# chhylp123/hifiasm

Measured on AMD Instinct MI355X. Metric: read-pair overlaps/sec (sum ol->length / (ha_pt_gen + all-reads h_ec_lchain pass)), higher is better.
Workload: dtype u64 hashing / int32 + f64 chain scores

## Files before the change

### hifiasm_amd/api.py

```python
from __future__ import annotations

import ctypes as C
import os

import numpy as np

_HERE = os.path.dirname(os.path.abspath(__file__))
_LIB = None


SORTDBG_SEQ, SORTDBG_WAVE_LDS, SORTDBG_WAVE_GLOBAL, SORTDBG_BLOCK, SORTDBG_SELECT = range(5)


class HaoError(RuntimeError):
    pass


class Opt(C.Structure):
    _fields_ = [("k", C.c_int32), ("w", C.c_int32), ("hpc", C.c_int32), ("sample_dist", C.c_int32), ("rewin", C.c_int32),
                ("min_hist_cnt", C.c_int32), ("max_kmer_cnt", C.c_int32), ("max_n_chain", C.c_int32),
                ("high_factor", C.c_double), ("is_ont", C.c_int32), ("bf_shift", C.c_int32), ("hg_size", C.c_int64)]


class Pass(C.Structure):
# ... 28 lines not shown


class WlistDelivery(C.Structure):
    _fields_ = [("n_ol", C.c_uint64), ("n_wins", C.c_uint64), ("n_cigar", C.c_uint64), ("n_swept", C.c_uint64), ("n_replace", C.c_uint64), ("n_untraced", C.c_uint64),
                ("win_off", C.c_void_p), ("wins", C.c_void_p), ("cig_off", C.c_void_p), ("cigars", C.c_void_p)]


DELIVER_OL, DELIVER_CL, DELIVER_EXACT, DELIVER_ED, DELIVER_TRACE, DELIVER_RESCUE, DELIVER_WLIST = 1, 2, 4, 8, 16, 32, 64
PLACE_DIAG, PLACE_REF = 0, 1

ABI_SYMBOLS = [
    "hao_opt_default", "hao_create", "hao_destroy", "hao_last_error", "hao_set_reads", "hao_ft_gen", "hao_pt_gen",
    "hao_ft_cnt", "hao_pt_get", "hao_ft_table", "hao_pt_table", "hao_hist", "hao_stats", "hao_sketch_batch",
    "hao_fetch_sketch", "hao_overlap_batch", "hao_fetch_seed_hits", "hao_fetch_overlaps", "hao_batch_totals", "hao_batch_seed_path", "hao_batch_chain_path",
    "hao_stage_times", "hao_pass_default", "hao_overlap_batch_ex", "hao_set_shard", "hao_dist_unique_id", "hao_dist_init",
    "hao_loop_create", "hao_loop_destroy", "hao_dist_init_loopback", "hao_batch_digest", "hao_selftest_rocprim", "hao_selftest_big", "hao_selftest_sortbits", "hao_unpack_cigar", "hao_unpack_overlaps", "hao_overlap_batch_async", "hao_deliver_wait", "hao_unpack_hits", "hao_exact_check", "hao_fetch_exact", "hao_window_ed_batch", "hao_index_save", "hao_index_load", "hao_next_slot", "hao_attach", "hao_window_trace_batch", "hao_delivery_digest", "hao_ft_passes", "hao_ovlp_bin_read", "hao_ovlp_bin_write", "hao_window_ed_grid", "hao_fetch_ed_grid",
    "hao_deliver_ed_config", "hao_deliver_ed", "hao_unpack_ed",
    "hao_window_trace_grid", "hao_fetch_trace_grid", "hao_deliver_trace", "hao_unpack_trace",
    "hao_window_ed_ref", "hao_fetch_ed_ovlp", "hao_deliver_ed_config_ref", "hao_ref_thresholds",
    "hao_window_rescue_ref", "hao_fetch_rescue", "hao_rescue_task", "hao_deliver_rescue", "hao_unpack_rescue",
    "hao_window_wlist_ref", "hao_fetch_wlist", "hao_deliver_wlist", "hao_unpack_wlist",
    "hao_dist_gather_reads", "hao_reads_digest", "hao_index_load_dist", "hao_shard_layout",
]


RESCUE_OVLP = np.dtype([("verdict", np.uint16), ("flags", np.uint16), ("exit_win", np.uint32), ("align_length", np.uint32), ("n_rescued", np.uint32)])
RESCUE_FWD, RESCUE_BWD, RESCUE_ANCHOR, RESCUE_UNTRACED, RESCUE_NO_EXIT = 0, 1, 2, 1, 0xFFFFFFFF
WLIST_PRIMARY, WLIST_UNTRACED = 3, 1 << 19


def wlist_records(raw):
# ... 635 lines not shown
```

### hifiasm_amd/csrc/hao_capi_rest.hpp

```cpp
#pragma once

#include <atomic>
#include <new>
#include <stdexcept>
#include <thread>
extern "C" {

int hao_ft_gen(hao_ctx *c, int32_t *hom_cov)
{
	if (!c) return HAO_EINVAL;
	HAO_NOT_ON_VIEW(c, "hao_ft_gen"); ++c->index_gen;
	HIP_TRY(hipSetDevice(c->device));
	c->timer.begin(c->stream);
	int rc = hao_ft_run(c);
	if (rc != HAO_OK) return rc;
	c->timer.mark("ft_release");
	HIP_TRY(hipStreamSynchronize(c->stream));
	c->timer.collect(c->stage_ms);
	if (hom_cov) *hom_cov = c->ft_peak_hom;
	return HAO_OK;
}

int32_t hao_ft_cnt(hao_ctx *c, uint64_t y)
{
// ... 692 lines not shown
	HAO_CHECK_LAUNCH();
	HIP_TRY(hipMemcpyAsync(out, d.p, n * 8, hipMemcpyDeviceToHost, c->stream));
	if (out_kh) HIP_TRY(hipMemcpyAsync(out_kh, d.p + n, n * 8, hipMemcpyDeviceToHost, c->stream));
	HIP_TRY(hipStreamSynchronize(c->stream));
	return HAO_OK;
}

__global__ void hao_selftest_fill_kernel(uint64_t n, uint64_t *x, uint64_t *v)
{
	const uint64_t i = (uint64_t)blockIdx.x * blockDim.x + threadIdx.x;
	if (i < n) { x[i] = hao_hash64(i * 0x9E3779B97F4A7C15ULL + 12345); v[i] = i; }
}
__global__ void hao_selftest_s40_fill_kernel(uint64_t n, uint64_t *x)
{
	const uint64_t i = (uint64_t)blockIdx.x * blockDim.x + threadIdx.x;
	if (i < n) { const uint64_t g = i % (n / 5 + 1); x[i] = (hao_hash64(g + 99) & ~((1ULL << HAO_SORT40_LOWBITS) - 1)) | ((g & 255) ? 0x155ULL : ((hao_hash64(i) >> 7) & 3) * 0x2a5b7ULL); }
}
__global__ void hao_selftest_s40_cmp_kernel(const uint64_t *a, const uint64_t *b, const uint32_t *ia, const uint32_t *ib, uint64_t n, unsigned long long *bad)
{
	const uint64_t i = (uint64_t)blockIdx.x * blockDim.x + threadIdx.x;
	if (i < n && (a[i] != b[i] || ia[i] != ib[i])) atomicAdd(bad, 1ULL);
}
int hao_selftest_sortbits(hao_ctx *c, uint64_t n, uint64_t out[4])
{
	if (!c || !out || n < 16 || n >= (1ULL << 32)) return HAO_EINVAL;
	HIP_TRY(hipSetDevice(c->device));
	DevBuf<uint64_t> x, s1, s2; DevBuf<uint32_t> o, o1, o2; DevBuf<unsigned long long> bad;
	HIP_TRY(x.reserve(n)); HIP_TRY(s1.reserve(n)); HIP_TRY(s2.reserve(n)); HIP_TRY(o.reserve(n)); HIP_TRY(o1.reserve(n)); HIP_TRY(o2.reserve(n)); HIP_TRY(bad.reserve(1));
	HIP_TRY(hipMemsetAsync(bad.p, 0, 8, c->stream));
	hipLaunchKernelGGL(hao_selftest_s40_fill_kernel, dim3((unsigned)((n + 255) / 256)), dim3(256), 0, c->stream, n, x.p); HAO_CHECK_LAUNCH();
	int rc = hao_index_sort(c, x.p, s1.p, o.p, o1.p, n, false);
	if (!rc) rc = hao_index_sort(c, x.p, s2.p, o.p, o2.p, n, true);
	if (!rc) {
		hipLaunchKernelGGL(hao_selftest_s40_cmp_kernel, dim3((unsigned)((n + 255) / 256)), dim3(256), 0, c->stream, s1.p, s2.p, o1.p, o2.p, n, bad.p);
		unsigned long long hb = 0;
		if (hipMemcpyAsync(&hb, bad.p, 8, hipMemcpyDeviceToHost, c->stream) != hipSuccess || hipStreamSynchronize(c->stream) != hipSuccess) rc = HAO_ENODEV;
		out[0] = hb; for (int k = 0; k < 3; ++k) out[1 + k] = c->peeked(PK_SORT40, k);
	}
	return rc;
}

int hao_selftest_rocprim(uint64_t n, uint64_t out[2])
{
	hao_ctx tmp_ctx; hao_ctx *c = &tmp_ctx;
	if (!out || n == 0 || n >= (1ULL << 32)) return HAO_EINVAL;
	out[0] = out[1] = 0;
	hipStream_t st = nullptr;
	DevBuf<uint64_t> x, v, x2, v2, gx, gv; DevBuf<uint32_t> ok, ok2, oi, oi2; DevBuf<unsigned char> tmp;
	HIP_TRY(x.reserve(n)); HIP_TRY(v.reserve(n)); HIP_TRY(x2.reserve(n)); HIP_TRY(v2.reserve(n)); HIP_TRY(gx.reserve(n)); HIP_TRY(gv.reserve(n));
	HIP_TRY(ok.reserve(n)); HIP_TRY(ok2.reserve(n)); HIP_TRY(oi.reserve(n)); HIP_TRY(oi2.reserve(n));
	hipLaunchKernelGGL(hao_selftest_fill_kernel, dim3((unsigned)((n + 255) / 256)), dim3(256), 0, st, n, x.p, v.p);
	HIP_TRY(hipGetLastError());
	size_t tb = 0;
	HIP_TRY(rocprim::radix_sort_pairs(nullptr, tb, x.p, x2.p, v.p, v2.p, n, 48, 64, st)); HIP_TRY(tmp.reserve(tb + 256));
// ... 65 lines not shown
```

### hifiasm_amd/csrc/hao_ctx.hpp

```cpp
#pragma once
#include <time.h>
#include <rocprim/rocprim.hpp>
#include <map>
#include <algorithm>
#include <cstdlib>
#include <cstring>
#include "hao_common.cuh"
#include "hao_grid_pair.cuh"

struct hao_ctx;
static void hao_set_err(hao_ctx *c, const std::string &m);

template<typename T> struct DevBuf {
	T *p = nullptr; size_t cap = 0; bool borrowed = false;
	DevBuf() = default;
	DevBuf(const DevBuf&) = delete; DevBuf &operator=(const DevBuf&) = delete;
	DevBuf(DevBuf &&o) noexcept : p(o.p), cap(o.cap), borrowed(o.borrowed) { o.p = nullptr; o.cap = 0; o.borrowed = false; }
	DevBuf &operator=(DevBuf &&o) noexcept { if (this != &o) { release(); p = o.p; cap = o.cap; borrowed = o.borrowed; o.p = nullptr; o.cap = 0; o.borrowed = false; } return *this; }
	~DevBuf() { release(); }
	hipError_t reserve(size_t n) {
		if (n <= cap) return hipSuccess;
		if (borrowed) return hipErrorInvalidValue;
		if (p) (void)hipFree(p);
		p = nullptr; cap = 0;
// ... 23 lines not shown
	void mark(const char *name) {
		size_t i = names.size();
		if (i >= ev.size()) { hipEvent_t e; (void)hipEventCreate(&e); ev.push_back(e); }
		names.push_back(name); host_t.push_back(now()); (void)hipEventRecord(ev[i], st);
		if (hao_dbg_sync) { const hipError_t e = hipStreamSynchronize(st); fprintf(stderr, "[stage] %s: %s\n", name, hipGetErrorString(e)); fflush(stderr); }
	}
	void collect(std::vector<std::pair<std::string, float> > &out) {
		out.clear();
		for (size_t i = 1; i < names.size(); ++i) { float ms = 0; (void)hipEventElapsedTime(&ms, ev[i - 1], ev[i]); out.push_back(std::make_pair(names[i], ms)); }
		for (size_t i = 1; i < names.size(); ++i) if (names[i].compare(0, 3, "ft_") == 0) out.push_back(std::make_pair("host_" + names[i], (float)((host_t[i] - host_t[i - 1]) * 1e3)));
	}
	~StageTimer() { for (auto e : ev) (void)hipEventDestroy(e); }
};

struct hao_switches {
	bool seedphase = false, qcphase = false, dp_stats = false, selphase = false, dltime = false, bloom = false;
	bool seq_chain = false, dp_seqtail = false, dp_nospec = false, dp_serial = false, seq_prune = false, seed_noql = false;
	long long sk_gcap = -1, exc_cap = -1, ft_chunk_slots = 0; unsigned long long gather_chunk = 64ULL << 20, ix_pad = 0, sort40_min = 1ULL << 23; int fc_raw_every = 0, exc_every = 0; bool qmz_raw = false, arena_probe = false;
	int arena_numa = 3, seed_merge_maxn = 24000, seed_lds_ratio = 120, ft_passes = 0, seed_lds = 1;
	static bool in_list(const char *v, const char *name) {
		const size_t n = strlen(name);
		for (const char *p = v; p && *p; ) { const char *e = strchr(p, ','); const size_t l = e ? (size_t)(e - p) : strlen(p); if (l == n && strncmp(p, name, n) == 0) return true; p = e ? e + 1 : nullptr; }
		return false;
	}
	static bool in_kv(const char *v, const char *name, unsigned long long &out) {
		const size_t n = strlen(name);
		for (const char *p = v; p && *p; ) { const char *e = strchr(p, ','); if (strncmp(p, name, n) == 0 && p[n] == '=') { out = strtoull(p + n + 1, nullptr, 10); return true; } p = e ? e + 1 : nullptr; }
		return false;
	}
	void load() {
		if (const char *v = getenv("HAO_DBG_PRINT")) {
			seedphase = in_list(v, "seed"); qcphase = in_list(v, "qc"); dp_stats = in_list(v, "dp"); selphase = in_list(v, "sel"); dltime = in_list(v, "dl"); bloom = in_list(v, "bloom"); hao_dbg_sync = in_list(v, "sync");
		}
		if (const char *v = getenv("HAO_DBG_FORCE")) {
			seq_chain = in_list(v, "seq_chain");
			dp_seqtail = in_list(v, "dp_seqtail");
			dp_nospec = in_list(v, "dp_nospec");
			dp_serial = in_list(v, "dp_serial");
			seq_prune = in_list(v, "seq_prune");
			seed_noql = in_list(v, "noql");
		}
		if (const char *v = getenv("HAO_DBG_TEST")) {
			unsigned long long x;
			if (in_kv(v, "ix_pad", x)) ix_pad = x;
			if (in_kv(v, "sort40_min", x)) sort40_min = x;
			if (in_kv(v, "sk_gcap", x)) sk_gcap = (long long)x;
			if (in_kv(v, "exc_cap", x)) exc_cap = (long long)x;
			if (in_kv(v, "fc_raw_every", x)) fc_raw_every = (int)x;
			if (in_kv(v, "exc_every", x)) exc_every = (int)x;
			if (in_kv(v, "qmz_raw", x)) qmz_raw = x != 0;
			if (in_kv(v, "arena_probe", x)) arena_probe = x != 0;
			if (in_kv(v, "ft_chunk_slots", x)) ft_chunk_slots = (long long)x;
			if (in_kv(v, "gather_chunk", x)) gather_chunk = std::max<unsigned long long>(x, 64);
		}
		if (const char *e = getenv("HAO_SEED_LDS")) seed_lds = atoi(e) ? 1 : 0;
		if (const char *e = getenv("HAO_SEED_LDS_RATIO")) seed_lds_ratio = std::max(0, atoi(e));
		if (const char *e = getenv("HAO_SEED_MERGE_MAXN")) seed_merge_maxn = std::max(0, atoi(e));
		if (const char *e = getenv("HAO_FT_PASSES")) ft_passes = std::max(0, atoi(e));
		if (const char *e = getenv("HAO_ARENA_NUMA")) arena_numa = atoi(e);
	}
// ... 83 lines not shown
	DevBuf<uint8_t> d_scalar_flag; DevBuf<uint32_t> d_scalar_list, d_unit_rid;
	DevBuf<uint64_t> d_pool_x, d_pool_info; DevBuf<uint32_t> d_pool_ord; DevBuf<unsigned long long> d_cursor; DevBuf<int> d_err;
	DevBuf<uint64_t> d_chunk_base, d_chunk_dst; DevBuf<uint32_t> d_chunk_cnt;
	DevBuf<uint64_t> d_g_x, d_g_info; DevBuf<uint32_t> d_g_ord; DevBuf<uint64_t> d_g_off; DevBuf<uint32_t> d_new_n; DevBuf<uint64_t> d_new_n64;
	DevBuf<uint64_t> d_mz_x, d_mz_info, d_mz_off;
	DevBuf<unsigned char> d_tmp; DevBuf<unsigned char> d_ring; DevBuf<uint32_t> d_ringord, d_cnt_ws;
	std::vector<uint64_t> h_mz_off; std::vector<hao_mz_t> h_mz_fetch;
	bool has_pt = false; int64_t pt_hist[HAO_N_COUNTS];
	uint64_t ix_n_mz = 0, ix_n_sorted = 0, ix_n_keys = 0, ix_n_pos = 0, ix_pad = 0; int ix_bucket_bits = 16;
	DevBuf<uint64_t> d_ix_mz_x, d_ix_mz_info, d_ix_mz_off;
	DevBuf<uint64_t> d_ix_sx, d_ix_sinfo;
	DevBuf<uint64_t> d_ix_lk; bool lk_valid = false; DevBuf<uint32_t> w_runid;
	DevBuf<uint64_t> d_ix_keys, d_ix_start; DevBuf<uint32_t> d_ix_cnt; DevBuf<uint32_t> d_ix_bucket;
	DevBuf<uint64_t> w_ukeys, w_flag, w_kpos, w_ustart; DevBuf<uint32_t> w_ucnt; DevBuf<unsigned long long> w_hist; DevBuf<uint32_t> w_ok, w_ok2, w_oi, w_oi2;
	DevBuf<uint32_t> w_s40_list, w_s40_o; DevBuf<uint64_t> w_s40_x, w_lkv2; DevBuf<unsigned long long> w_s40_cnt; uint64_t s40_runs = 0;
	std::vector<uint64_t> h_ix_keys, h_ix_off, h_ix_pos, h_ix_mz_off; bool h_ix_valid = false;
	WinResident win;
	DevBuf<hao_ed_task_t> al_task; DevBuf<uint64_t> al_k1, al_k2, al_path; DevBuf<uint32_t> al_i1, al_order, al_sel; DevBuf<hao_ed_result_t> al_res; DevBuf<hao_trace_result_t> al_tres;
	DevBuf<uint8_t> al_want; DevBuf<uint16_t> al_cig;
	uint32_t ded_window = 0, ded_thre = 0;
	uint32_t ded_place = 0; double ded_erate = 0; DevBuf<uint8_t> ded_tab;
	struct RefGrid {
		DevBuf<uint64_t> cnt, woff; DevBuf<int16_t> shift; DevBuf<uint8_t> werr; DevBuf<hao_ed_pair> pairs; DevBuf<unsigned long long> ctr;
	} rf;
	DevBuf<uint8_t> rf_tab; uint32_t rf_tab_wl = 0; double rf_tab_erate = 0; DevBuf<hao_ed_ovlp_sum> rf_sum; std::vector<hao_ed_ovlp_sum> rf_hsum; uint64_t rf_unres = 0, rs_wc = 0;
	struct Rescue {
		DevBuf<uint16_t> wpe; DevBuf<uint64_t> rbase, path, off; DevBuf<hao_rs_state> st; DevBuf<hao_rs_win> rec, wins; DevBuf<hao_rs_ovlp> ovlp; DevBuf<unsigned long long> ctr;
		std::vector<hao_rs_ovlp> h_ovlp; std::vector<uint64_t> h_win_off; std::vector<hao_rs_win> h_wins;
	} rs;
	uint64_t rs_slots = 0, rs_rounds = 0, rs_active = 0, rs_total = 0, rs_nw = 0;
// ... 77 lines not shown
```

### hifiasm_amd/csrc/hao_index.cuh

```cuda
#pragma once
#include "hao_common.cuh"
#include "hao_sketch.cuh"

#define HAO_KH_CHUNK 2048

struct hao_kh_args {
	const uint8_t *packed; const uint64_t *pk_off; const uint32_t *len;
	const uint64_t *tile_off; const uint32_t *tile_ord; const uint32_t *n_runs;
	const uint64_t *chunk_off; const uint8_t *scalar_flag; const uint64_t *kmer_off;
	uint64_t rid_lo, n_sel; int k, hpc; uint64_t *out;
	uint64_t ch0;
};

__global__ __launch_bounds__(256) void kmer_hash_chunk_kernel(hao_kh_args a)
{
	extern __shared__ __align__(16) unsigned char smem[];
	const int k = a.k, tid = threadIdx.x, lane = tid & 63, wv = tid >> 6;
	const int NE = HAO_KH_CHUNK + k + 1, NW = (NE + 63) / 64 + 1;
	uint64_t *pl0 = (uint64_t*)smem, *pl1 = pl0 + NW; uint8_t *rcode = (uint8_t*)(pl1 + NW);
	uint64_t ch = blockIdx.x + a.ch0, lo = 0, hi = a.n_sel;
	while (lo < hi) { uint64_t m = (lo + hi) >> 1; if (a.chunk_off[m + 1] <= ch) lo = m + 1; else hi = m; }
	const uint64_t r = lo;
	if (a.scalar_flag[r]) return;
	const uint32_t ci = (uint32_t)(ch - a.chunk_off[r]);
// ... 103 lines not shown
__global__ void hao_bucket_kernel(const uint64_t *keys, uint64_t n, int shift, uint32_t nb, uint32_t *bucket)
{
	uint32_t b = blockIdx.x * blockDim.x + threadIdx.x;
	if (b > nb) return;
	if (b == nb) { bucket[b] = (uint32_t)n; return; }
	uint64_t lo = 0, hi = n;
	while (lo < hi) { uint64_t m = (lo + hi) >> 1; if ((keys[m] >> shift) < b) lo = m + 1; else hi = m; }
	bucket[b] = (uint32_t)lo;
}

__global__ void hao_iota_kernel(uint32_t *v, uint64_t n)
{
	const uint64_t i = (uint64_t)blockIdx.x * blockDim.x + threadIdx.x;
	if (i < n) v[i] = (uint32_t)i;
}
#define HAO_SORT40_LOWBITS 24
__global__ void hao_sort40_mark_kernel(const uint64_t *sx, uint64_t m, uint32_t *list, unsigned long long *cnt, uint64_t cap)
{
	const uint64_t j = (uint64_t)blockIdx.x * blockDim.x + threadIdx.x + 1;
	if (j >= m) return;
	const uint64_t b = sx[j], a = sx[j - 1], top = b >> HAO_SORT40_LOWBITS;
	if ((a >> HAO_SORT40_LOWBITS) != top || a <= b) return;
	uint64_t i = j - 1;
	while (i > 0 && (sx[i - 1] >> HAO_SORT40_LOWBITS) == top) { if (sx[i - 1] > sx[i]) return; --i; }
	const unsigned long long k = atomicAdd(cnt, 1ULL);
	if (k < cap) list[k] = (uint32_t)i;
}
__global__ __launch_bounds__(64) void hao_sort40_fix_kernel(uint64_t *sx, uint32_t *oi, uint64_t m, const uint32_t *list, unsigned long long *cnt, uint64_t cap, uint64_t *tx, uint32_t *to, uint64_t tcap)
{
	const uint64_t n_runs = cnt[0] < cap ? cnt[0] : cap;
	if (blockIdx.x >= n_runs) return;
	const int lane = hao_lane();
	const uint64_t s = list[blockIdx.x], top = sx[s] >> HAO_SORT40_LOWBITS;
	uint64_t e = s;
	for (;;) {
		const uint64_t i = e + lane; const unsigned long long bal = __ballot(i < m && (sx[i] >> HAO_SORT40_LOWBITS) == top);
		if (bal == ~0ULL) { e += 64; continue; }
		e += (uint64_t)(__ffsll((long long)~bal) - 1); break;
	}
	const uint64_t L = e - s;
	unsigned long long base = 0;
	if (lane == 0) base = atomicAdd(cnt + 1, (unsigned long long)L);
	base = (unsigned long long)__shfl((long long)base, 0);
	if (base + L > tcap) { if (lane == 0) cnt[2] = 1; return; }
	uint64_t last = 0, out = 0; bool first = true;
	while (out < L) {
		uint64_t mn = ~0ULL;
		for (uint64_t i = s + lane; i < e; i += 64) { const uint64_t k = sx[i]; if ((first || k > last) && k < mn) mn = k; }
#pragma unroll
		for (int d = 32; d >= 1; d >>= 1) { const uint64_t o = (uint64_t)__shfl_xor((long long)mn, d); if (o < mn) mn = o; }
		for (uint64_t i0 = s; i0 < e; i0 += 64) {
// ... 15 lines not shown
	const uint32_t o = sidx[j], u = runid[j] - 1;
	sinfo[j] = info[o];
	int c = ucnt[u] > HAO_MAX_COUNT ? HAO_MAX_COUNT : (int)ucnt[u];
	lk[o] = (c >= lo && c <= hi) ? ((ustart[u] + base) | (uint64_t)c << 48) : 0;
}
__global__ void hao_index_gather_kernel(uint64_t m, const uint32_t *sidx, const uint32_t *runid, const uint32_t *ucnt, const uint64_t *ustart, int lo, int hi,
		const uint64_t *info, uint64_t *sinfo, uint64_t *val, uint64_t base)
{
	const uint64_t j = (uint64_t)blockIdx.x * blockDim.x + threadIdx.x;
	if (j >= m) return;
	const uint32_t o = sidx[j], u = runid[j] - 1;
	sinfo[j] = info[o];
	int c = ucnt[u] > HAO_MAX_COUNT ? HAO_MAX_COUNT : (int)ucnt[u];
	val[j] = (c >= lo && c <= hi) ? ((ustart[u] + base) | (uint64_t)c << 48) : 0;
}
__global__ void hao_scatter_u64_kernel(const uint64_t *in, const uint32_t *idx, uint64_t n, uint64_t *out)
{
	const uint64_t i = (uint64_t)blockIdx.x * blockDim.x + threadIdx.x;
	if (i < n) out[idx[i]] = in[i];
}

struct hao_pt_dev {
	const uint64_t *keys, *start; const uint32_t *cnt, *bucket; const uint64_t *sinfo; uint64_t n_keys; int bshift;
};

__device__ __forceinline__ uint32_t hao_pt_lookup(const hao_pt_dev &pt, uint64_t x, uint64_t *start)
{
	uint32_t b = (uint32_t)(x >> pt.bshift), lo = pt.bucket[b], hi = pt.bucket[b + 1], e = hi;
	while (lo < hi) { uint32_t m = (lo + hi) >> 1; if (pt.keys[m] < x) lo = m + 1; else hi = m; }
	if (lo < e && pt.keys[lo] == x) { *start = pt.start[lo]; return pt.cnt[lo]; }
// ... 33 lines not shown
```

### hifiasm_amd/csrc/hao_tables.hpp

```cpp
#pragma once
#include <chrono>
#include "hao_comm.hpp"
#include "hao_pipeline.hpp"
#include "hao_index.cuh"
#include "hao_host.hpp"

__global__ void hao_lower_bound_kernel(const uint64_t *keys, uint64_t n, const uint64_t *targets, int nt, uint64_t *out)
{
	int t = blockIdx.x * blockDim.x + threadIdx.x;
	if (t >= nt) return;
	uint64_t lo = 0, hi = n, x = targets[t];
	while (lo < hi) { uint64_t m = (lo + hi) >> 1; if (keys[m] < x) lo = m + 1; else hi = m; }
	out[t] = lo;
}
__global__ void hao_lower_bound_low12_kernel(const uint64_t *keys, uint64_t n, const uint64_t *targets, int nt, uint64_t *out)
{
	int t = blockIdx.x * blockDim.x + threadIdx.x;
	if (t >= nt) return;
	uint64_t lo = 0, hi = n, x = targets[t];
	while (lo < hi) { uint64_t m = (lo + hi) >> 1; if ((keys[m] & 4095) < x) lo = m + 1; else hi = m; }
	out[t] = lo;
}
__global__ void hao_owner_key_kernel(const uint64_t *x, uint64_t n, uint32_t *key, uint32_t *idx)
{
// ... 531 lines not shown
	if (int rc = hao_build_bucket(c, c->d_ft_keys.p, n_kept, 16, c->d_ft_bucket)) return rc;
	if (int rc = hao_ft_build_hash(c, n_kept)) return rc;
	HIP_TRY(hipStreamSynchronize(c->stream));
	kcnt.release(); slots.release(); chunks.release(); kmer_off.release(); kh_chunk_off.release();
	c->has_ft = true;
	{
		int mx = (int)(c->ft_peak_hom * c->opt.high_factor + .499);
		c->hom_cov = c->ft_peak_hom;
		if (c->max_n_chain < mx) c->max_n_chain = mx;
	}
	c->timer.mark("ft_table");
	return HAO_OK;
}

static inline uint64_t hao_sort40_cap(uint64_t m) { return std::max<uint64_t>(1 << 16, m >> 10); }
static int hao_index_sort(hao_ctx *c, const uint64_t *x, uint64_t *sx, uint32_t *oi, uint32_t *oi2, uint64_t m, bool sort40)
{
	hipLaunchKernelGGL(hao_iota_kernel, dim3((unsigned)((m + 255) / 256)), dim3(256), 0, c->stream, oi, m); HAO_CHECK_LAUNCH();
	const int b0 = sort40 ? HAO_SORT40_LOWBITS : 0;
	size_t tb = 0;
	HIP_TRY(rocprim::radix_sort_pairs(nullptr, tb, x, sx, oi, oi2, m, b0, 64, c->stream)); HIP_TRY(hao_tmp(c, tb));
	HIP_TRY(rocprim::radix_sort_pairs(c->d_tmp.p, tb, x, sx, oi, oi2, m, b0, 64, c->stream));
	if (sort40) {
		const uint64_t cap = hao_sort40_cap(m), tcap = 64 * cap;
		HIP_TRY(c->w_s40_list.reserve(cap)); HIP_TRY(c->w_s40_x.reserve(tcap)); HIP_TRY(c->w_s40_o.reserve(tcap)); HIP_TRY(c->w_s40_cnt.reserve(4));
		HIP_TRY(hipMemsetAsync(c->w_s40_cnt.p, 0, 32, c->stream));
		hipLaunchKernelGGL(hao_sort40_mark_kernel, dim3((unsigned)((m + 255) / 256)), dim3(256), 0, c->stream, sx, m, c->w_s40_list.p, c->w_s40_cnt.p, cap); HAO_CHECK_LAUNCH();
		hipLaunchKernelGGL(hao_sort40_fix_kernel, dim3((unsigned)cap), dim3(64), 0, c->stream, sx, oi2, m, c->w_s40_list.p, c->w_s40_cnt.p, cap, c->w_s40_x.p, c->w_s40_o.p, tcap); HAO_CHECK_LAUNCH();
		if (int rc = hao_peek(c, c->w_s40_cnt.p, 3, PK_SORT40)) return rc;
	}
	return HAO_OK;
}

static int hao_pt_run(hao_ctx *c)
{
	const uint64_t n = c->n_reads;
	c->has_pt = false; c->h_ix_valid = false; c->h_ix_mz_off.clear();
	const bool sharded = c->comm && c->comm->active();
	auto local_sketch = [&]() -> int {
		if (n == 0) { hao_set_err(c, "no reads"); return HAO_EINVAL; }
		if (int rc = hao_sketch_run(c, 0, n, c->has_ft, c->opt.sample_dist, 1)) return rc;
		std::swap(c->d_ix_mz_x, c->d_mz_x); std::swap(c->d_ix_mz_info, c->d_mz_info); std::swap(c->d_ix_mz_off, c->d_mz_off);
		HIP_TRY(c->d_mz_x.reserve_exact(c->d_ix_mz_x.cap)); HIP_TRY(c->d_mz_info.reserve_exact(c->d_ix_mz_info.cap)); HIP_TRY(c->d_mz_off.reserve_exact(c->d_ix_mz_off.cap));
// ... 20 lines not shown
		return HAO_OK;
	};
	auto peaks_and_range = [&](int *hi_out) {
		int het = -1;
		c->hom_cov = hao_find_peaks(c->pt_hist, HAO_N_COUNTS, c->opt.min_hist_cnt, &het, hao_prior_hom(c)); c->het_cov = het;
		int hi;
		if (c->has_ft) hi = HAO_MAX_COUNT - 1;
		else { hi = (int)(c->hom_cov * c->opt.high_factor); if (hi > HAO_MAX_COUNT - 1) hi = HAO_MAX_COUNT - 1; }
		*hi_out = hi;
	};
	c->lk_valid = false;
	if (!sharded) {
		const uint64_t m = c->ix_n_mz;
		if (m >= (1ULL << 32)) { hao_set_err(c, "more than 2^32 minimizers on one device"); return HAO_EUNSUPP; }
		const uint64_t pad = c->ix_pad = c->sw.ix_pad;
		HIP_TRY(c->d_ix_sx.reserve(m + 1)); HIP_TRY(c->d_ix_sinfo.reserve(m + pad + 8)); HIP_TRY(c->w_oi.reserve(m + 1)); HIP_TRY(c->w_oi2.reserve(m + 1));
		HIP_TRY(c->w_runid.reserve(m + 1)); HIP_TRY(c->d_ix_lk.reserve(m + 1));
		bool sort40 = m >= c->sw.sort40_min;
		for (;;) {
			if (m) { if (int rc = hao_index_sort(c, c->d_ix_mz_x.p, c->d_ix_sx.p, c->w_oi.p, c->w_oi2.p, m, sort40)) return rc; }
			c->ix_n_sorted = m;
			c->timer.mark("pt_sort");
			if (int rc = rle_hist(c->d_ix_sx.p, m)) return rc;
			if (m && sort40) {
				c->s40_runs = c->peeked(PK_SORT40);
				if (c->s40_runs > hao_sort40_cap(m) || c->peeked(PK_SORT40, 2)) { sort40 = false; continue; }
			}
			break;
		}
		c->timer.mark("pt_count");
		int hi; peaks_and_range(&hi);
		if (int rc = hao_keep_runs(c, ukeys.p, ucnt.p, n_unique, 2, hi, c->d_ix_keys, &c->d_ix_start, c->d_ix_cnt, &c->ix_n_keys, &c->ix_n_pos)) return rc;
		if (m) {
			auto heads = rocprim::make_transform_iterator(rocprim::make_counting_iterator<uint64_t>(0), RunHead32{c->d_ix_sx.p});
			size_t tb = 0;
			HIP_TRY(rocprim::inclusive_scan(nullptr, tb, heads, c->w_runid.p, m, rocprim::plus<uint32_t>(), c->stream)); HIP_TRY(hao_tmp(c, tb));
			HIP_TRY(rocprim::inclusive_scan(c->d_tmp.p, tb, heads, c->w_runid.p, m, rocprim::plus<uint32_t>(), c->stream));
			if (m >= c->sw.sort40_min) {
				int nb = 1; while ((1ULL << nb) < m) ++nb;
				const int b0 = nb > 8 ? nb - 8 : 0;
				HIP_TRY(c->w_lkv2.reserve(m + 1));
				hipLaunchKernelGGL(hao_index_gather_kernel, dim3((unsigned)((m + 255) / 256)), dim3(256), 0, c->stream, m, c->w_oi2.p, c->w_runid.p, ucnt.p, c->w_ustart.p, 2, hi,
								   c->d_ix_mz_info.p, c->d_ix_sinfo.p + pad, c->d_ix_sx.p, pad);
				HAO_CHECK_LAUNCH();
				size_t tb2 = 0;
				HIP_TRY(rocprim::radix_sort_pairs(nullptr, tb2, c->w_oi2.p, c->w_oi.p, c->d_ix_sx.p, c->w_lkv2.p, m, b0, nb, c->stream)); HIP_TRY(hao_tmp(c, tb2));
				HIP_TRY(rocprim::radix_sort_pairs(c->d_tmp.p, tb2, c->w_oi2.p, c->w_oi.p, c->d_ix_sx.p, c->w_lkv2.p, m, b0, nb, c->stream));
				hipLaunchKernelGGL(hao_scatter_u64_kernel, dim3((unsigned)((m + 255) / 256)), dim3(256), 0, c->stream, c->w_lkv2.p, c->w_oi.p, m, c->d_ix_lk.p);
				HAO_CHECK_LAUNCH();
			} else {
				hipLaunchKernelGGL(hao_index_finish_kernel, dim3((unsigned)((m + 255) / 256)), dim3(256), 0, c->stream, m, c->w_oi2.p, c->w_runid.p, ucnt.p, c->w_ustart.p, 2, hi,
								   c->d_ix_mz_info.p, c->d_ix_sinfo.p + pad, c->d_ix_lk.p, pad);
				HAO_CHECK_LAUNCH();
			}
			if (pad && c->ix_n_keys) { hipLaunchKernelGGL(hao_add_const_kernel, dim3((unsigned)((c->ix_n_keys + 255) / 256)), dim3(256), 0, c->stream, c->d_ix_start.p, c->ix_n_keys, pad); HAO_CHECK_LAUNCH(); }
		}
		c->lk_valid = true;
// ... 158 lines not shown
```

### include/hao.h

```cpp
#ifndef HAO_H
#define HAO_H
#include <stdint.h>

#ifdef __cplusplus
extern "C" {
#endif

#define HAO_OK          0
#define HAO_ENODEV     -1
#define HAO_EINVAL     -2
#define HAO_ENOMEM     -3
#define HAO_EUNSUPP    -4

typedef struct hao_ctx hao_ctx;

typedef struct {
	int32_t k;
	int32_t w;
	int32_t hpc;
	int32_t sample_dist;
	int32_t rewin;
	int32_t min_hist_cnt;
	int32_t max_kmer_cnt;
	int32_t max_n_chain;
// ... 199 lines not shown
int hao_index_load(hao_ctx *c, const char *prefix, int32_t *number_of_round);
int hao_index_load_dist(hao_ctx *c, const char *prefix, const uint64_t *first_rid , int32_t *number_of_round);
int hao_shard_layout(hao_ctx *c, uint64_t *n_reads, uint64_t *rid_base, uint64_t *n_total, const uint32_t **all_len);

typedef struct { uint64_t qns; uint32_t qe, tn, ts, te; uint32_t ml, rev, bl, del; uint8_t el, no_l_indel, pad[6]; } hao_ma_hit_t;
int hao_ovlp_bin_read(const char *path, uint64_t *n_reads, uint8_t **flags, uint64_t **off, hao_ma_hit_t **hits);
int hao_ovlp_bin_write(const char *path, uint64_t n_reads, const uint8_t *flags, const uint64_t *off, const hao_ma_hit_t *hits);

int hao_batch_digest(hao_ctx *c, uint64_t *out, uint64_t *out_kh);
int hao_delivery_digest(const hao_delivery_t *d, uint64_t *out, int n_threads);

int hao_selftest_rocprim(uint64_t n, uint64_t out[2]);
int hao_selftest_big(uint64_t n, uint64_t out[3]);

int hao_selftest_sortbits(hao_ctx *c, uint64_t n, uint64_t out[4]);

#define HAO_SORTDBG_SEQ 0
#define HAO_SORTDBG_WAVE_LDS 1
#define HAO_SORTDBG_WAVE_GLOBAL 2
#define HAO_SORTDBG_BLOCK 3
#define HAO_SORTDBG_SELECT 4
int hao_dbg_sort_perm(hao_ctx *c, int mode, int path, int variant, uint64_t n_arr, const uint64_t *off, const uint64_t *xs, const int32_t *sc, uint32_t *perm);

int hao_stage_times(hao_ctx *c, const char **names, float *ms, int cap);

#ifdef __cplusplus
}
#endif
#endif
```

Before: 179.7 million.

## Adaptive partial-key radix sort ladder and run-walk index gather

The index sort now picks how many low key bits to skip (32, 24 or 0) using a collision estimate taken from the previous build or the k-mer peak. If the fix-up pass overflows, it falls back one rung at a time. For large indexes with many distinct keys, a new per-run kernel assigns run info by binary search over run starts in shared memory. This replaces the inclusive scan that built run ids and the per-element gather. The aim is to cut radix passes and a full scan over all minimizers, at the risk of retries when the estimate is wrong. Selftests and debug switches are also added.

```diff
diff --git a/hifiasm_amd/api.py b/hifiasm_amd/api.py
--- a/hifiasm_amd/api.py
+++ b/hifiasm_amd/api.py
@@ -66,7 +66,7 @@
     "hao_ft_cnt", "hao_pt_get", "hao_ft_table", "hao_pt_table", "hao_hist", "hao_stats", "hao_sketch_batch",
     "hao_fetch_sketch", "hao_overlap_batch", "hao_fetch_seed_hits", "hao_fetch_overlaps", "hao_batch_totals", "hao_batch_seed_path", "hao_batch_chain_path",
     "hao_stage_times", "hao_pass_default", "hao_overlap_batch_ex", "hao_set_shard", "hao_dist_unique_id", "hao_dist_init",
-    "hao_loop_create", "hao_loop_destroy", "hao_dist_init_loopback", "hao_batch_digest", "hao_selftest_rocprim", "hao_selftest_big", "hao_selftest_sortbits", "hao_unpack_cigar", "hao_unpack_overlaps", "hao_overlap_batch_async", "hao_deliver_wait", "hao_unpack_hits", "hao_exact_check", "hao_fetch_exact", "hao_window_ed_batch", "hao_index_save", "hao_index_load", "hao_next_slot", "hao_attach", "hao_window_trace_batch", "hao_delivery_digest", "hao_ft_passes", "hao_ovlp_bin_read", "hao_ovlp_bin_write", "hao_window_ed_grid", "hao_fetch_ed_grid",
+    "hao_loop_create", "hao_loop_destroy", "hao_dist_init_loopback", "hao_batch_digest", "hao_selftest_rocprim", "hao_selftest_big", "hao_selftest_sortbits", "hao_selftest_sortladder", "hao_selftest_index_runs", "hao_unpack_cigar", "hao_unpack_overlaps", "hao_overlap_batch_async", "hao_deliver_wait", "hao_unpack_hits", "hao_exact_check", "hao_fetch_exact", "hao_window_ed_batch", "hao_index_save", "hao_index_load", "hao_next_slot", "hao_attach", "hao_window_trace_batch", "hao_delivery_digest", "hao_ft_passes", "hao_ovlp_bin_read", "hao_ovlp_bin_write", "hao_window_ed_grid", "hao_fetch_ed_grid",
     "hao_deliver_ed_config", "hao_deliver_ed", "hao_unpack_ed",
     "hao_window_trace_grid", "hao_fetch_trace_grid", "hao_deliver_trace", "hao_unpack_trace",
     "hao_window_ed_ref", "hao_fetch_ed_ovlp", "hao_deliver_ed_config_ref", "hao_ref_thresholds",
diff --git a/hifiasm_amd/csrc/hao_capi_rest.hpp b/hifiasm_amd/csrc/hao_capi_rest.hpp
--- a/hifiasm_amd/csrc/hao_capi_rest.hpp
+++ b/hifiasm_amd/csrc/hao_capi_rest.hpp
@@ -730,7 +730,7 @@
 __global__ void hao_selftest_s40_fill_kernel(uint64_t n, uint64_t *x)
 {
 	const uint64_t i = (uint64_t)blockIdx.x * blockDim.x + threadIdx.x;
-	if (i < n) { const uint64_t g = i % (n / 5 + 1); x[i] = (hao_hash64(g + 99) & ~((1ULL << HAO_SORT40_LOWBITS) - 1)) | ((g & 255) ? 0x155ULL : ((hao_hash64(i) >> 7) & 3) * 0x2a5b7ULL); }
+	if (i < n) { const uint64_t g = i % (n / 5 + 1); x[i] = (hao_hash64(g + 99) & ~((1ULL << 24) - 1)) | ((g & 255) ? 0x155ULL : ((hao_hash64(i) >> 7) & 3) * 0x2a5b7ULL); }
 }
 __global__ void hao_selftest_s40_cmp_kernel(const uint64_t *a, const uint64_t *b, const uint32_t *ia, const uint32_t *ib, uint64_t n, unsigned long long *bad)
 {
@@ -743,10 +743,11 @@
 	HIP_TRY(hipSetDevice(c->device));
 	DevBuf<uint64_t> x, s1, s2; DevBuf<uint32_t> o, o1, o2; DevBuf<unsigned long long> bad;
 	HIP_TRY(x.reserve(n)); HIP_TRY(s1.reserve(n)); HIP_TRY(s2.reserve(n)); HIP_TRY(o.reserve(n)); HIP_TRY(o1.reserve(n)); HIP_TRY(o2.reserve(n)); HIP_TRY(bad.reserve(1));
+	const uint64_t cap = hao_sort40_cap(n);
 	HIP_TRY(hipMemsetAsync(bad.p, 0, 8, c->stream));
 	hipLaunchKernelGGL(hao_selftest_s40_fill_kernel, dim3((unsigned)((n + 255) / 256)), dim3(256), 0, c->stream, n, x.p); HAO_CHECK_LAUNCH();
-	int rc = hao_index_sort(c, x.p, s1.p, o.p, o1.p, n, false);
-	if (!rc) rc = hao_index_sort(c, x.p, s2.p, o.p, o2.p, n, true);
+	int rc = hao_index_sort(c, x.p, s1.p, o.p, o1.p, n, 0, cap, 64 * cap);
+	if (!rc) rc = hao_index_sort(c, x.p, s2.p, o.p, o2.p, n, 24, cap, 64 * cap);
 	if (!rc) {
 		hipLaunchKernelGGL(hao_selftest_s40_cmp_kernel, dim3((unsigned)((n + 255) / 256)), dim3(256), 0, c->stream, s1.p, s2.p, o1.p, o2.p, n, bad.p);
 		unsigned long long hb = 0;
@@ -754,6 +755,69 @@
 		out[0] = hb; for (int k = 0; k < 3; ++k) out[1 + k] = c->peeked(PK_SORT40, k);
 	}
 	return rc;
+}
+
+__global__ void hao_selftest_ladder_fill_kernel(uint64_t n, int lowbits, uint64_t *x)
+{
+	const uint64_t i = (uint64_t)blockIdx.x * blockDim.x + threadIdx.x;
+	if (i >= n) return;
+	const uint64_t G = n / 5 + 1, g = i % G, k = i / G, top = (g * 0x9E3779B97F4A7C15ULL) & (~0ULL >> lowbits);
+	uint64_t low = 0x155;
+	if ((g & 255) == 0) { const int p = (int)((g >> 8) % 3); low = (p == 0 ? ((k & 1) ? 1 : 2) : p == 1 ? (k % 3 ? k % 3 : 3) : ((0x31524 >> (4 * k)) & 15)) * 0x2a5b7ULL; }
+	x[i] = top << lowbits | low;
+}
+int hao_selftest_sortladder(hao_ctx *c, const uint64_t *keys, uint64_t n, int lowbits, uint64_t cap, uint64_t tcap, uint64_t *out_keys, uint32_t *out_idx, uint64_t out[6])
+{
+	if (!c || !out || n < 16 || n >= (1ULL << 32) || (lowbits != 0 && lowbits != 24 && lowbits != 32) || (!keys && !lowbits)) return HAO_EINVAL;
+	HIP_TRY(hipSetDevice(c->device));
+	if (!cap) cap = hao_sort40_cap(n);
+	if (!tcap) tcap = 64 * cap;
+	if (cap >= (1ULL << 31)) return HAO_EINVAL;
+	DevBuf<uint64_t> x, s1, s2; DevBuf<uint32_t> o, o1, o2; DevBuf<unsigned long long> bad;
+	HIP_TRY(x.reserve(n)); HIP_TRY(s1.reserve(n)); HIP_TRY(s2.reserve(n)); HIP_TRY(o.reserve(n)); HIP_TRY(o1.reserve(n)); HIP_TRY(o2.reserve(n)); HIP_TRY(bad.reserve(1));
+	HIP_TRY(hipMemsetAsync(bad.p, 0, 8, c->stream));
+	if (keys) HIP_TRY(hipMemcpyAsync(x.p, keys, n * 8, hipMemcpyHostToDevice, c->stream));
+	else { hipLaunchKernelGGL(hao_selftest_ladder_fill_kernel, dim3((unsigned)((n + 255) / 256)), dim3(256), 0, c->stream, n, lowbits, x.p); HAO_CHECK_LAUNCH(); }
+	if (int rc = hao_index_sort(c, x.p, s1.p, o.p, o1.p, n, 0, cap, tcap)) return rc;
+	uint64_t retries = 0;
+	for (int k = 0; k < 4; ++k) out[k] = 0;
+	for (;;) {
+		if (int rc = hao_index_sort(c, x.p, s2.p, o.p, o2.p, n, lowbits, cap, tcap)) return rc;
+		HIP_TRY(hipStreamSynchronize(c->stream));
+		if (!lowbits) break;
+		for (int k = 0; k < 3; ++k) out[1 + k] = c->peeked(PK_SORT40, k);
+		if (!hao_sort_failed(c, cap)) break;
+		lowbits = hao_sort_next_rung(lowbits); ++retries;
+	}
+	out[4] = (uint64_t)lowbits; out[5] = retries;
+	hipLaunchKernelGGL(hao_selftest_s40_cmp_kernel, dim3((unsigned)((n + 255) / 256)), dim3(256), 0, c->stream, s1.p, s2.p, o1.p, o2.p, n, bad.p); HAO_CHECK_LAUNCH();
+	unsigned long long hb = 0;
+	HIP_TRY(hipMemcpyAsync(&hb, bad.p, 8, hipMemcpyDeviceToHost, c->stream));
+	if (out_keys) HIP_TRY(hipMemcpyAsync(out_keys, s2.p, n * 8, hipMemcpyDeviceToHost, c->stream));
+	if (out_idx) HIP_TRY(hipMemcpyAsync(out_idx, o2.p, n * 4, hipMemcpyDeviceToHost, c->stream));
+	HIP_TRY(hipStreamSynchronize(c->stream));
+	out[0] = hb;
+	return HAO_OK;
+}
+
+int hao_selftest_index_runs(hao_ctx *c, uint64_t m, uint64_t n_runs, const uint64_t *ustart, const uint32_t *ucnt, int lo, int hi, uint64_t pad, const uint32_t *sidx, const uint64_t *info,
+		uint64_t *out_sinfo, uint64_t *out_val)
+{
+	if (!c || !m || !n_runs || n_runs > m || m >= (1ULL << 32) || !ustart || !ucnt || !sidx || !info || !out_sinfo || !out_val || lo < 1 || ustart[0] != 0) return HAO_EINVAL;
+	for (uint64_t u = 0; u < n_runs; ++u) if (ustart[u] >= m || (u && ustart[u] <= ustart[u - 1])) { hao_set_err(c, "hao_selftest_index_runs: run starts do not ascend inside the positions"); return HAO_EINVAL; }
+	for (uint64_t j = 0; j < m; ++j) if (sidx[j] >= m) { hao_set_err(c, "hao_selftest_index_runs: a carried index beyond the records"); return HAO_EINVAL; }
+	HIP_TRY(hipSetDevice(c->device));
+	DevBuf<uint64_t> d_st, d_info, d_sinfo, d_val; DevBuf<uint32_t> d_cnt, d_sidx;
+	HIP_TRY(d_st.reserve(n_runs + 1)); HIP_TRY(d_cnt.reserve(n_runs + 1)); HIP_TRY(d_sidx.reserve(m)); HIP_TRY(d_info.reserve(m)); HIP_TRY(d_sinfo.reserve(m + pad)); HIP_TRY(d_val.reserve(m));
+	HIP_TRY(hipMemcpyAsync(d_st.p, ustart, n_runs * 8, hipMemcpyHostToDevice, c->stream)); HIP_TRY(hipMemcpyAsync(d_cnt.p, ucnt, n_runs * 4, hipMemcpyHostToDevice, c->stream));
+	HIP_TRY(hipMemcpyAsync(d_sidx.p, sidx, m * 4, hipMemcpyHostToDevice, c->stream)); HIP_TRY(hipMemcpyAsync(d_info.p, info, m * 8, hipMemcpyHostToDevice, c->stream));
+	HIP_TRY(hipMemsetAsync(d_sinfo.p, 0xff, (m + pad) * 8, c->stream)); HIP_TRY(hipMemsetAsync(d_val.p, 0xff, m * 8, c->stream));
+	hipLaunchKernelGGL(hao_index_runs_kernel, dim3((unsigned)((n_runs + HAO_IXR_RUNS - 1) / HAO_IXR_RUNS)), dim3(256), 0, c->stream, m, n_runs, d_sidx.p, d_cnt.p, d_st.p, lo, hi,
+					   d_info.p, d_sinfo.p + pad, d_val.p, pad);
+	HAO_CHECK_LAUNCH();
+	HIP_TRY(hipMemcpyAsync(out_sinfo, d_sinfo.p + pad, m * 8, hipMemcpyDeviceToHost, c->stream)); HIP_TRY(hipMemcpyAsync(out_val, d_val.p, m * 8, hipMemcpyDeviceToHost, c->stream));
+	HIP_TRY(hipStreamSynchronize(c->stream));
+	return HAO_OK;
 }
 
 int hao_selftest_rocprim(uint64_t n, uint64_t out[2])
diff --git a/hifiasm_amd/csrc/hao_ctx.hpp b/hifiasm_amd/csrc/hao_ctx.hpp
--- a/hifiasm_amd/csrc/hao_ctx.hpp
+++ b/hifiasm_amd/csrc/hao_ctx.hpp
@@ -61,9 +61,9 @@
 };
 
 struct hao_switches {
-	bool seedphase = false, qcphase = false, dp_stats = false, selphase = false, dltime = false, bloom = false;
+	bool seedphase = false, qcphase = false, dp_stats = false, selphase = false, dltime = false, bloom = false, sortprint = false;
 	bool seq_chain = false, dp_seqtail = false, dp_nospec = false, dp_serial = false, seq_prune = false, seed_noql = false;
-	long long sk_gcap = -1, exc_cap = -1, ft_chunk_slots = 0; unsigned long long gather_chunk = 64ULL << 20, ix_pad = 0, sort40_min = 1ULL << 23; int fc_raw_every = 0, exc_every = 0; bool qmz_raw = false, arena_probe = false;
+	long long sk_gcap = -1, exc_cap = -1, ft_chunk_slots = 0; unsigned long long gather_chunk = 64ULL << 20, ix_pad = 0, sort40_min = 1ULL << 23, ixr_min = 0; int fc_raw_every = 0, exc_every = 0, sort_lowbits = -1; bool qmz_raw = false, arena_probe = false;
 	int arena_numa = 3, seed_merge_maxn = 24000, seed_lds_ratio = 120, ft_passes = 0, seed_lds = 1;
 	static bool in_list(const char *v, const char *name) {
 		const size_t n = strlen(name);
@@ -77,7 +77,7 @@
 	}
 	void load() {
 		if (const char *v = getenv("HAO_DBG_PRINT")) {
-			seedphase = in_list(v, "seed"); qcphase = in_list(v, "qc"); dp_stats = in_list(v, "dp"); selphase = in_list(v, "sel"); dltime = in_list(v, "dl"); bloom = in_list(v, "bloom"); hao_dbg_sync = in_list(v, "sync");
+			seedphase = in_list(v, "seed"); qcphase = in_list(v, "qc"); dp_stats = in_list(v, "dp"); selphase = in_list(v, "sel"); dltime = in_list(v, "dl"); bloom = in_list(v, "bloom"); sortprint = in_list(v, "sort"); hao_dbg_sync = in_list(v, "sync");
 		}
 		if (const char *v = getenv("HAO_DBG_FORCE")) {
 			seq_chain = in_list(v, "seq_chain");
@@ -91,6 +91,8 @@
 			unsigned long long x;
 			if (in_kv(v, "ix_pad", x)) ix_pad = x;
 			if (in_kv(v, "sort40_min", x)) sort40_min = x;
+			if (in_kv(v, "sort_lowbits", x)) sort_lowbits = (int)x;
+			if (in_kv(v, "ixr_min", x)) ixr_min = x;
 			if (in_kv(v, "sk_gcap", x)) sk_gcap = (long long)x;
 			if (in_kv(v, "exc_cap", x)) exc_cap = (long long)x;
 			if (in_kv(v, "fc_raw_every", x)) fc_raw_every = (int)x;
@@ -204,6 +206,7 @@
 	DevBuf<uint64_t> d_ix_keys, d_ix_start; DevBuf<uint32_t> d_ix_cnt; DevBuf<uint32_t> d_ix_bucket;
 	DevBuf<uint64_t> w_ukeys, w_flag, w_kpos, w_ustart; DevBuf<uint32_t> w_ucnt; DevBuf<unsigned long long> w_hist; DevBuf<uint32_t> w_ok, w_ok2, w_oi, w_oi2;
 	DevBuf<uint32_t> w_s40_list, w_s40_o; DevBuf<uint64_t> w_s40_x, w_lkv2; DevBuf<unsigned long long> w_s40_cnt; uint64_t s40_runs = 0;
+	int s40_lowbits = 0; uint64_t s40_prev_m = 0, s40_prev_unique = 0;
 	std::vector<uint64_t> h_ix_keys, h_ix_off, h_ix_pos, h_ix_mz_off; bool h_ix_valid = false;
 	WinResident win;
 	DevBuf<hao_ed_task_t> al_task; DevBuf<uint64_t> al_k1, al_k2, al_path; DevBuf<uint32_t> al_i1, al_order, al_sel; DevBuf<hao_ed_result_t> al_res; DevBuf<hao_trace_result_t> al_tres;
diff --git a/hifiasm_amd/csrc/hao_index.cuh b/hifiasm_amd/csrc/hao_index.cuh
--- a/hifiasm_amd/csrc/hao_index.cuh
+++ b/hifiasm_amd/csrc/hao_index.cuh
@@ -141,27 +141,26 @@
 	const uint64_t i = (uint64_t)blockIdx.x * blockDim.x + threadIdx.x;
 	if (i < n) v[i] = (uint32_t)i;
 }
-#define HAO_SORT40_LOWBITS 24
-__global__ void hao_sort40_mark_kernel(const uint64_t *sx, uint64_t m, uint32_t *list, unsigned long long *cnt, uint64_t cap)
+__global__ void hao_sort40_mark_kernel(const uint64_t *sx, uint64_t m, uint32_t *list, unsigned long long *cnt, uint64_t cap, int lowbits)
 {
 	const uint64_t j = (uint64_t)blockIdx.x * blockDim.x + threadIdx.x + 1;
 	if (j >= m) return;
-	const uint64_t b = sx[j], a = sx[j - 1], top = b >> HAO_SORT40_LOWBITS;
-	if ((a >> HAO_SORT40_LOWBITS) != top || a <= b) return;
+	const uint64_t b = sx[j], a = sx[j - 1], top = b >> lowbits;
+	if ((a >> lowbits) != top || a <= b) return;
 	uint64_t i = j - 1;
-	while (i > 0 && (sx[i - 1] >> HAO_SORT40_LOWBITS) == top) { if (sx[i - 1] > sx[i]) return; --i; }
+	while (i > 0 && (sx[i - 1] >> lowbits) == top) { if (sx[i - 1] > sx[i]) return; --i; }
 	const unsigned long long k = atomicAdd(cnt, 1ULL);
 	if (k < cap) list[k] = (uint32_t)i;
 }
-__global__ __launch_bounds__(64) void hao_sort40_fix_kernel(uint64_t *sx, uint32_t *oi, uint64_t m, const uint32_t *list, unsigned long long *cnt, uint64_t cap, uint64_t *tx, uint32_t *to, uint64_t tcap)
+__global__ __launch_bounds__(64) void hao_sort40_fix_kernel(uint64_t *sx, uint32_t *oi, uint64_t m, const uint32_t *list, unsigned long long *cnt, uint64_t cap, uint64_t *tx, uint32_t *to, uint64_t tcap, int lowbits)
 {
 	const uint64_t n_runs = cnt[0] < cap ? cnt[0] : cap;
 	if (blockIdx.x >= n_runs) return;
 	const int lane = hao_lane();
-	const uint64_t s = list[blockIdx.x], top = sx[s] >> HAO_SORT40_LOWBITS;
+	const uint64_t s = list[blockIdx.x], top = sx[s] >> lowbits;
 	uint64_t e = s;
 	for (;;) {
-		const uint64_t i = e + lane; const unsigned long long bal = __ballot(i < m && (sx[i] >> HAO_SORT40_LOWBITS) == top);
+		const uint64_t i = e + lane; const unsigned long long bal = __ballot(i < m && (sx[i] >> lowbits) == top);
 		if (bal == ~0ULL) { e += 64; continue; }
 		e += (uint64_t)(__ffsll((long long)~bal) - 1); break;
 	}
@@ -207,6 +206,26 @@
 	int c = ucnt[u] > HAO_MAX_COUNT ? HAO_MAX_COUNT : (int)ucnt[u];
 	val[j] = (c >= lo && c <= hi) ? ((ustart[u] + base) | (uint64_t)c << 48) : 0;
 }
+#define HAO_IXR_RUNS 256
+__global__ __launch_bounds__(256) void hao_index_runs_kernel(uint64_t m, uint64_t n_runs, const uint32_t *sidx, const uint32_t *ucnt, const uint64_t *ustart, int lo, int hi,
+		const uint64_t *info, uint64_t *sinfo, uint64_t *val, uint64_t base)
+{
+	__shared__ uint64_t l_start[HAO_IXR_RUNS + 1]; __shared__ uint32_t l_cnt[HAO_IXR_RUNS];
+	const uint64_t u0 = (uint64_t)blockIdx.x * HAO_IXR_RUNS;
+	if (u0 >= n_runs) return;
+	const int R = (int)(n_runs - u0 < HAO_IXR_RUNS ? n_runs - u0 : HAO_IXR_RUNS);
+	for (int t = threadIdx.x; t <= R; t += 256) l_start[t] = u0 + t < n_runs ? ustart[u0 + t] : m;
+	for (int t = threadIdx.x; t < R; t += 256) { const int c = ucnt[u0 + t] > HAO_MAX_COUNT ? HAO_MAX_COUNT : (int)ucnt[u0 + t]; l_cnt[t] = (c >= lo && c <= hi) ? (uint32_t)c : 0u; }
+	__syncthreads();
+	const uint64_t j1 = l_start[R] < m ? l_start[R] : m;
+	for (uint64_t j = l_start[0] + threadIdx.x; j < j1; j += 256) {
+		int a = 0, b = R;
+		while (b - a > 1) { const int mid = (a + b) >> 1; if (l_start[mid] <= j) a = mid; else b = mid; }
+		sinfo[j] = info[sidx[j]];
+		const uint64_t c = l_cnt[a];
+		val[j] = c ? ((l_start[a] + base) | c << 48) : 0;
+	}
+}
 __global__ void hao_scatter_u64_kernel(const uint64_t *in, const uint32_t *idx, uint64_t n, uint64_t *out)
 {
 	const uint64_t i = (uint64_t)blockIdx.x * blockDim.x + threadIdx.x;
diff --git a/hifiasm_amd/csrc/hao_tables.hpp b/hifiasm_amd/csrc/hao_tables.hpp
--- a/hifiasm_amd/csrc/hao_tables.hpp
+++ b/hifiasm_amd/csrc/hao_tables.hpp
@@ -569,19 +569,29 @@
 }
 
 static inline uint64_t hao_sort40_cap(uint64_t m) { return std::max<uint64_t>(1 << 16, m >> 10); }
-static int hao_index_sort(hao_ctx *c, const uint64_t *x, uint64_t *sx, uint32_t *oi, uint32_t *oi2, uint64_t m, bool sort40)
+static inline int hao_sort_next_rung(int lowbits) { return lowbits > 24 ? 24 : 0; }
+static inline bool hao_sort_failed(const hao_ctx *c, uint64_t cap) { return c->peeked(PK_SORT40) > cap || c->peeked(PK_SORT40, 2) != 0; }
+static int hao_sort_first_rung(const hao_ctx *c, uint64_t m)
+{
+	if (c->sw.sort_lowbits == 0 || c->sw.sort_lowbits == 24 || c->sw.sort_lowbits == 32) return c->sw.sort_lowbits;
+	double n = 0;
+	if (c->s40_prev_m && c->s40_prev_unique) n = (double)c->s40_prev_unique * ((double)m / (double)c->s40_prev_m);
+	else { const int peak = c->has_ft && c->ft_peak_hom > 0 ? c->ft_peak_hom : hao_prior_hom(c); if (peak >= 2) n = (double)m / peak + (double)m / 8; }
+	if (n <= 0) return 24;
+	const double crowd = std::max(1.0, 0.25 * (double)c->opt.w);
+	return n * n / 8589934592.0 * crowd <= 0.5 * (double)hao_sort40_cap(m) ? 32 : 24;
+}
+static int hao_index_sort(hao_ctx *c, const uint64_t *x, uint64_t *sx, uint32_t *oi, uint32_t *oi2, uint64_t m, int lowbits, uint64_t cap, uint64_t tcap)
 {
 	hipLaunchKernelGGL(hao_iota_kernel, dim3((unsigned)((m + 255) / 256)), dim3(256), 0, c->stream, oi, m); HAO_CHECK_LAUNCH();
-	const int b0 = sort40 ? HAO_SORT40_LOWBITS : 0;
 	size_t tb = 0;
-	HIP_TRY(rocprim::radix_sort_pairs(nullptr, tb, x, sx, oi, oi2, m, b0, 64, c->stream)); HIP_TRY(hao_tmp(c, tb));
-	HIP_TRY(rocprim::radix_sort_pairs(c->d_tmp.p, tb, x, sx, oi, oi2, m, b0, 64, c->stream));
-	if (sort40) {
-		const uint64_t cap = hao_sort40_cap(m), tcap = 64 * cap;
+	HIP_TRY(rocprim::radix_sort_pairs(nullptr, tb, x, sx, oi, oi2, m, lowbits, 64, c->stream)); HIP_TRY(hao_tmp(c, tb));
+	HIP_TRY(rocprim::radix_sort_pairs(c->d_tmp.p, tb, x, sx, oi, oi2, m, lowbits, 64, c->stream));
+	if (lowbits) {
 		HIP_TRY(c->w_s40_list.reserve(cap)); HIP_TRY(c->w_s40_x.reserve(tcap)); HIP_TRY(c->w_s40_o.reserve(tcap)); HIP_TRY(c->w_s40_cnt.reserve(4));
 		HIP_TRY(hipMemsetAsync(c->w_s40_cnt.p, 0, 32, c->stream));
-		hipLaunchKernelGGL(hao_sort40_mark_kernel, dim3((unsigned)((m + 255) / 256)), dim3(256), 0, c->stream, sx, m, c->w_s40_list.p, c->w_s40_cnt.p, cap); HAO_CHECK_LAUNCH();
-		hipLaunchKernelGGL(hao_sort40_fix_kernel, dim3((unsigned)cap), dim3(64), 0, c->stream, sx, oi2, m, c->w_s40_list.p, c->w_s40_cnt.p, cap, c->w_s40_x.p, c->w_s40_o.p, tcap); HAO_CHECK_LAUNCH();
+		hipLaunchKernelGGL(hao_sort40_mark_kernel, dim3((unsigned)((m + 255) / 256)), dim3(256), 0, c->stream, sx, m, c->w_s40_list.p, c->w_s40_cnt.p, cap, lowbits); HAO_CHECK_LAUNCH();
+		hipLaunchKernelGGL(hao_sort40_fix_kernel, dim3((unsigned)cap), dim3(64), 0, c->stream, sx, oi2, m, c->w_s40_list.p, c->w_s40_cnt.p, cap, c->w_s40_x.p, c->w_s40_o.p, tcap, lowbits); HAO_CHECK_LAUNCH();
 		if (int rc = hao_peek(c, c->w_s40_cnt.p, 3, PK_SORT40)) return rc;
 	}
 	return HAO_OK;
@@ -632,33 +642,45 @@
 		const uint64_t m = c->ix_n_mz;
 		if (m >= (1ULL << 32)) { hao_set_err(c, "more than 2^32 minimizers on one device"); return HAO_EUNSUPP; }
 		const uint64_t pad = c->ix_pad = c->sw.ix_pad;
+		const bool big = m >= c->sw.sort40_min;
 		HIP_TRY(c->d_ix_sx.reserve(m + 1)); HIP_TRY(c->d_ix_sinfo.reserve(m + pad + 8)); HIP_TRY(c->w_oi.reserve(m + 1)); HIP_TRY(c->w_oi2.reserve(m + 1));
-		HIP_TRY(c->w_runid.reserve(m + 1)); HIP_TRY(c->d_ix_lk.reserve(m + 1));
-		bool sort40 = m >= c->sw.sort40_min;
+		HIP_TRY(c->d_ix_lk.reserve(m + 1));
+		int lowbits = big ? hao_sort_first_rung(c, m) : 0, retries = 0;
+		const uint64_t cap = hao_sort40_cap(m);
 		for (;;) {
-			if (m) { if (int rc = hao_index_sort(c, c->d_ix_mz_x.p, c->d_ix_sx.p, c->w_oi.p, c->w_oi2.p, m, sort40)) return rc; }
+			if (m) { if (int rc = hao_index_sort(c, c->d_ix_mz_x.p, c->d_ix_sx.p, c->w_oi.p, c->w_oi2.p, m, lowbits, cap, 64 * cap)) return rc; }
 			c->ix_n_sorted = m;
 			c->timer.mark("pt_sort");
 			if (int rc = rle_hist(c->d_ix_sx.p, m)) return rc;
-			if (m && sort40) {
+			if (m && lowbits) {
 				c->s40_runs = c->peeked(PK_SORT40);
-				if (c->s40_runs > hao_sort40_cap(m) || c->peeked(PK_SORT40, 2)) { sort40 = false; continue; }
+				if (c->sw.sortprint) fprintf(stderr, "[sort40] m = %llu: rung %d, %llu dirty runs listed (list holds %llu), %llu scratch elements used (of %llu), overflow %llu\n", (unsigned long long)m, lowbits,
+					(unsigned long long)c->s40_runs, (unsigned long long)cap, (unsigned long long)c->peeked(PK_SORT40, 1), (unsigned long long)(64 * cap), (unsigned long long)c->peeked(PK_SORT40, 2));
+				if (hao_sort_failed(c, cap)) { lowbits = hao_sort_next_rung(lowbits); ++retries; continue; }
 			}
 			break;
 		}
+		c->s40_lowbits = lowbits; c->s40_prev_m = m; c->s40_prev_unique = n_unique;
+		if (c->sw.sortprint) fprintf(stderr, "[sort40] m = %llu: %llu distinct keys, sorted on rung %d after %d retries\n", (unsigned long long)m, (unsigned long long)n_unique, lowbits, retries);
 		c->timer.mark("pt_count");
 		int hi; peaks_and_range(&hi);
 		if (int rc = hao_keep_runs(c, ukeys.p, ucnt.p, n_unique, 2, hi, c->d_ix_keys, &c->d_ix_start, c->d_ix_cnt, &c->ix_n_keys, &c->ix_n_pos)) return rc;
 		if (m) {
-			auto heads = rocprim::make_transform_iterator(rocprim::make_counting_iterator<uint64_t>(0), RunHead32{c->d_ix_sx.p});
-			size_t tb = 0;
-			HIP_TRY(rocprim::inclusive_scan(nullptr, tb, heads, c->w_runid.p, m, rocprim::plus<uint32_t>(), c->stream)); HIP_TRY(hao_tmp(c, tb));
-			HIP_TRY(rocprim::inclusive_scan(c->d_tmp.p, tb, heads, c->w_runid.p, m, rocprim::plus<uint32_t>(), c->stream));
-			if (m >= c->sw.sort40_min) {
+			const bool walk = big && n_unique >= (c->sw.ixr_min ? c->sw.ixr_min : 1024ULL * HAO_IXR_RUNS);
+			if (!walk) {
+				HIP_TRY(c->w_runid.reserve(m + 1));
+				auto heads = rocprim::make_transform_iterator(rocprim::make_counting_iterator<uint64_t>(0), RunHead32{c->d_ix_sx.p});
+				size_t tb = 0;
+				HIP_TRY(rocprim::inclusive_scan(nullptr, tb, heads, c->w_runid.p, m, rocprim::plus<uint32_t>(), c->stream)); HIP_TRY(hao_tmp(c, tb));
+				HIP_TRY(rocprim::inclusive_scan(c->d_tmp.p, tb, heads, c->w_runid.p, m, rocprim::plus<uint32_t>(), c->stream));
+			}
+			if (big) {
 				int nb = 1; while ((1ULL << nb) < m) ++nb;
 				const int b0 = nb > 8 ? nb - 8 : 0;
 				HIP_TRY(c->w_lkv2.reserve(m + 1));
-				hipLaunchKernelGGL(hao_index_gather_kernel, dim3((unsigned)((m + 255) / 256)), dim3(256), 0, c->stream, m, c->w_oi2.p, c->w_runid.p, ucnt.p, c->w_ustart.p, 2, hi,
+				if (walk) hipLaunchKernelGGL(hao_index_runs_kernel, dim3((unsigned)((n_unique + HAO_IXR_RUNS - 1) / HAO_IXR_RUNS)), dim3(256), 0, c->stream, m, n_unique, c->w_oi2.p, ucnt.p, c->w_ustart.p, 2, hi,
+								   c->d_ix_mz_info.p, c->d_ix_sinfo.p + pad, c->d_ix_sx.p, pad);
+				else hipLaunchKernelGGL(hao_index_gather_kernel, dim3((unsigned)((m + 255) / 256)), dim3(256), 0, c->stream, m, c->w_oi2.p, c->w_runid.p, ucnt.p, c->w_ustart.p, 2, hi,
 								   c->d_ix_mz_info.p, c->d_ix_sinfo.p + pad, c->d_ix_sx.p, pad);
 				HAO_CHECK_LAUNCH();
 				size_t tb2 = 0;
diff --git a/include/hao.h b/include/hao.h
--- a/include/hao.h
+++ b/include/hao.h
@@ -237,6 +237,9 @@
 int hao_selftest_big(uint64_t n, uint64_t out[3]);
 
 int hao_selftest_sortbits(hao_ctx *c, uint64_t n, uint64_t out[4]);
+int hao_selftest_sortladder(hao_ctx *c, const uint64_t *keys, uint64_t n, int lowbits, uint64_t cap, uint64_t tcap, uint64_t *out_keys, uint32_t *out_idx, uint64_t out[6]);
+int hao_selftest_index_runs(hao_ctx *c, uint64_t m, uint64_t n_runs, const uint64_t *ustart, const uint32_t *ucnt, int lo, int hi, uint64_t pad, const uint32_t *sidx, const uint64_t *info,
+		uint64_t *out_sinfo, uint64_t *out_val);
 
 #define HAO_SORTDBG_SEQ 0
 #define HAO_SORTDBG_WAVE_LDS 1
```

New measurement: 180.3 million (median of 4 runs). No clear change (+0.3%).
